# mlpc-ucsd/BDM

Hardware: AMD Instinct MI355X
Metric: sampled shapes/sec (4096 pts, 1000 DDPM steps) (higher is better)
Workload: dtype f32

## Files before the change

bdm_amd/csrc/dense_ops.hip:

```cpp
#include <stdlib.h>

#include "../../include/bdm_hip.h"
#include "common.h"
#include "se_fc.h"

using namespace bdm;
typedef __attribute__((ext_vector_type(16))) float f32x16;

#include "pointwise_common.h"

template <int MI, int NI, bool ATRANS = false, int BK = 16, bool FOLD = false>
__global__ __launch_bounds__(256) __attribute__((amdgpu_waves_per_eu(2))) void pw_gemm_kernel(int M, int K, int N, const float *__restrict__ W, int ldw,
                                                      long long bsw, const int *__restrict__ m_count,
                                                      const float *__restrict__ X, long long bsx, int ldx,
                                                      const float *__restrict__ bias,
                                                      const float *__restrict__ bbias, int ldbb,
                                                      const float *__restrict__ R, long long bsr, int ldr,
                                                      float *__restrict__ Y, long long bsy, int ldy, int act,
                                                      float slope, PwGn gn) {
  constexpr int BM = 32 * MI, BN = 128 * NI, LDA = BM + 4;
  __shared__ float As[BK * LDA];
  __shared__ __align__(16) float Bs[BK * BN];
  __shared__ float2 coef_s[FOLD ? 1024 : 1];
  const int tid = threadIdx.x, lane = tid & 63, wave = tid >> 6, li = lane & 31, lh = lane >> 5;
// ... 1042 lines not shown
  if (b == 0) return BDM_OK;
  if (workspace != nullptr) {
    const int p = sa_row_floats(c);
    BDM_REQUIRE((reinterpret_cast<size_t>(workspace) & 15) == 0, "sa_group: workspace must be 16-byte aligned");
    hipLaunchKernelGGL(sa_pack_points_kernel, dim3(cdiv(n, 256), cdiv(p / 4, 3), b), dim3(256), 0, (hipStream_t)stream, c, n, p,
                       coords, features, bs_f, ld_f, (float *)workspace);
    hipLaunchKernelGGL(sa_group_pm_kernel, dim3(cdiv(m * u, 256), cdiv(p / 4, SAQ), b), dim3(256), 0, (hipStream_t)stream, c,
                       n, m, u, p, (const float *)workspace, centers, indices, out);
    return launch_status("sa_group");
  }
  if (n >= 256 && n <= 8192 && (long long)m * u <= (1ll << 24)) {
    const int dma = (n % 256 == 0) && (ld_f % 4 == 0) && (bs_f % 4 == 0) && ((reinterpret_cast<size_t>(coords) & 15) == 0) &&
                    (c == 0 || (reinterpret_cast<size_t>(features) & 15) == 0);
    const size_t smem = sizeof(float) * SAG_R * (size_t)n + 1024;
    BDM_ALLOW_LDS(sa_group_lds_kernel, smem);
    hipLaunchKernelGGL(sa_group_lds_kernel, dim3(cdiv(c + 3, SAG_R), cdiv(m * u, SAG_EB), b), dim3(256), smem, (hipStream_t)stream, c, n, m, u,
                       dma, coords, centers, features, bs_f, ld_f, indices, out);
    return launch_status("sa_group");
  }
  int gy = c < 32 ? (c < 1 ? 1 : c) : 32;
  hipLaunchKernelGGL(sa_group_kernel, dim3(cdiv(m * u, 256), gy, b), dim3(256), 0, (hipStream_t)stream, c, n, m, u,
                     coords, centers, features, bs_f, ld_f, indices, out);
  return launch_status("sa_group");
}

__global__ void bcast_rows_kernel(int c, int l, const float *__restrict__ v, int ld_v, float *__restrict__ y,
                                  long long bs_y, int ld_y) {
  const int col = blockIdx.x * blockDim.x + threadIdx.x;
  const int bi = blockIdx.z;
  if (col >= l) return;
  for (int ci = blockIdx.y; ci < c; ci += gridDim.y)
    y[(size_t)bi * bs_y + (size_t)ci * ld_y + col] = v[(size_t)bi * ld_v + ci];
}
extern "C" int bdm_broadcast_rows(int b, int c, int l, const float *v, int ld_v, float *y, long long bs_y,
                                  int ld_y, void *stream) {
  BDM_REQUIRE(b >= 0 && c >= 1 && l >= 1, "broadcast_rows: bad sizes");
  if (b == 0) return BDM_OK;
  hipLaunchKernelGGL(bcast_rows_kernel, dim3(cdiv(l, 256), c < 64 ? c : 64, b), dim3(256), 0, (hipStream_t)stream, c,
                     l, v, ld_v, y, bs_y, ld_y);
  return launch_status("broadcast_rows");
}

__global__ void copy_rows_kernel(int c, int l, const float *__restrict__ x, long long bs_x, int ld_x,
                                 float *__restrict__ y, long long bs_y, int ld_y) {
  const int col = blockIdx.x * blockDim.x + threadIdx.x;
  const int bi = blockIdx.z;
// ... 682 lines not shown
```

bdm_amd/csrc/pvcnn_ops.hip:

```cpp
#include <stdarg.h>
#include <stdio.h>

#include <stdlib.h>

#include "../../include/bdm_hip.h"
#include "common.h"

#pragma clang fp contract(off)

namespace bdm {
static thread_local char g_err[512] = "";
void set_error(const char *fmt, ...) {
  va_list ap;
  va_start(ap, fmt);
  vsnprintf(g_err, sizeof(g_err), fmt, ap);
  va_end(ap);
}
}

extern "C" const char *bdm_last_error(void) { return bdm::g_err; }
extern "C" int bdm_abi_version(void) { return 4; }

using namespace bdm;

// ... 500 lines not shown
          __fadd_rn(__fadd_rn(__fmul_rn(fr[i0], w0), __fmul_rn(fr[i1], w1)), __fmul_rn(fr[i2], w2));
    } else if (ci < c_a + c_s) {
      out0[(size_t)bi * bs_0 + (size_t)ci * ld_0 + j] = fs[(size_t)bi * bs_s + (size_t)(ci - c_a) * ld_s + j];
    } else {
      const int ct = ci - c_a - c_s;
      const float *fr = ft + (size_t)bi * bs_t + (size_t)ct * ld_t;
      out1[(size_t)bi * bs_1 + (size_t)ct * ld_1 + j] =
          __fadd_rn(__fadd_rn(__fmul_rn(fr[i0], w0), __fmul_rn(fr[i1], w1)), __fmul_rn(fr[i2], w2));
    }
  }
}

extern "C" int bdm_fp_assemble(int b, int m, int n, const int *indices, const float *weights, int c_a, const float *fa,
                               long long bs_a, int ld_a, int c_s, const float *fs, long long bs_s, int ld_s, int c_t,
                               const float *ft, long long bs_t, int ld_t, float *out0, long long bs_0, int ld_0, float *out1,
                               long long bs_1, int ld_1, void *stream) {
  BDM_REQUIRE(b >= 0 && m >= 1 && n >= 0 && c_a >= 0 && c_s >= 0 && c_t >= 0, "fp_assemble: bad sizes");
  if (b == 0 || n == 0 || c_a + c_s + c_t == 0) return BDM_OK;
  const int c = c_a + c_s + c_t;
  dim3 grid(cdiv(n, 256), c < 64 ? c : 64, b);
  hipLaunchKernelGGL(fp_assemble_kernel, grid, dim3(256), 0, (hipStream_t)stream, n, c_a, fa, bs_a, ld_a, c_s, fs, bs_s, ld_s, c_t,
                     ft, bs_t, ld_t, indices, weights, out0, bs_0, ld_0, out1, bs_1, ld_1);
  return launch_status("fp_assemble");
}

extern "C" int bdm_three_nn_interpolate_forward(int b, int c, int m, int n, const float *points,
                                                const float *centers, const float *features, float *out,
                                                int *indices, float *weights, void *stream) {
  int rc = bdm_three_nn_search(b, m, n, points, centers, indices, weights, stream);
  if (rc) return rc;
  return bdm_three_nn_apply(b, c, m, n, features, (long long)c * m, m, indices, weights, out,
                            (long long)c * n, n, stream);
}

extern "C" size_t bdm_voxelize_workspace_bytes(int b, int n, int r) {
  return sizeof(int) * ((size_t)b * r * r * r + 2 * (size_t)b * n);
}

__global__ void vox_plan_kernel(int n, int r, const int *__restrict__ coords, int *__restrict__ ind,
                                int *__restrict__ cnt, int *__restrict__ start, int *__restrict__ tmp,
                                int *__restrict__ sorted, int n_max, int *__restrict__ occ_index,
                                int *__restrict__ occ_list, int *__restrict__ n_occ, unsigned char *__restrict__ rowocc) {
  extern __shared__ int lcnt[];
  __shared__ int wave_tot[16];
  const int r2 = r * r, r3 = r2 * r;
  const int bi = blockIdx.x, tid = threadIdx.x, T = blockDim.x, lane = tid & 63, wave = tid >> 6;
// ... 290 lines not shown
```

bdm_amd/modules.py:

```python
import os
from typing import NamedTuple

import torch
import torch.nn as nn

from . import functional as F
from . import ops
from . import tape

__all__ = ["Swish", "SharedMLP", "SE3d", "Voxelization", "Attention", "PVConv", "BallQuery",
           "PointNetSAModule", "PointNetFPModule"]


class Swish(nn.Module):

    def forward(self, x):
        raise RuntimeError("Swish is fused into bdm_group_norm on the HIP path")


class SharedMLP(nn.Module):

    def __init__(self, in_channels, out_channels, dim=1):
        super().__init__()
        if dim == 1:
            conv = nn.Conv1d
        elif dim == 2:
            conv = nn.Conv2d
        else:
            raise ValueError
        if not isinstance(out_channels, (list, tuple)):
            out_channels = [out_channels]
        layers = []
        for oc in out_channels:
            layers.extend([conv(in_channels, oc, 1), nn.GroupNorm(8, oc), Swish()])
            in_channels = oc
        self.layers = nn.Sequential(*layers)

    fold_gn = True

    def run(self, x, out_last=None, fold_last=False, x2=None, first_weight=None, first_add=None, first_bias=None):
        n = len(self.layers) // 3
        pending = None
        for i in range(n):
            conv, gn = self.layers[3 * i], self.layers[3 * i + 1]
            last = i == n - 1
            dst = out_last if last else None
            defer = (self.fold_gn and x.is_cuda and (not last or fold_last) and ops.gn_foldable(conv.out_channels, gn.num_groups))
            second = x2 if i == 0 else None
            weight = first_weight if (i == 0 and first_weight is not None) else conv.weight
            addend = first_add if i == 0 else None
            bb = first_bias if i == 0 else None
            if defer or pending is not None or second is not None or addend is not None or bb is not None:
                r = ops.pointwise_conv_gn(x, weight, conv.bias, out=dst, fold_in=pending,
                                          out_groups=gn.num_groups if defer else None, x2=second, add=addend, batch_bias=bb)
                if defer:
                    x, stats = r
                    pending = (stats, gn)
                else:
                    x, pending = r, None
                    ops.group_norm_(x, gn.weight, gn.bias, gn.num_groups, gn.eps, swish=True)
            else:
                x = ops.pointwise_conv(x, weight, conv.bias, out=dst)
                ops.group_norm_(x, gn.weight, gn.bias, gn.num_groups, gn.eps, swish=True)
        return (x, pending) if fold_last else x

    def forward(self, inputs):
        if isinstance(inputs, (list, tuple)):
            return (self.run(inputs[0]), *inputs[1:])
        return self.run(inputs)


def hoisted_first_weight(owner, conv, keep_cols):
    w = conv.weight
    hit = getattr(owner, "_hoist_w", None)
    if hit is None or hit[0] != (w._version, w.data_ptr(), keep_cols):
        w2 = w.detach().reshape(w.shape[0], -1)
        kept = w2[:, :keep_cols] if isinstance(keep_cols, int) else torch.cat([w2[:, lo:hi] for lo, hi in keep_cols], dim=1)
        hit = ((w._version, w.data_ptr(), keep_cols), kept.contiguous())
        owner._hoist_w = hit
    return hit[1]


class SE3d(nn.Module):

    def __init__(self, channel, reduction=8, use_relu=False):
        super().__init__()
        if not use_relu:
            raise NotImplementedError("the denoisers are built with with_se_relu=True (pvcnn_utils.py:93)")
        self.fc = nn.Sequential(nn.Linear(channel, channel // reduction, bias=False), nn.ReLU(True),
                                nn.Linear(channel // reduction, channel, bias=False), nn.Sigmoid())

    def gate(self, grid):
        return ops.se_gate(grid, self.fc[0].weight, self.fc[2].weight)


class Voxelization(nn.Module):

    def __init__(self, resolution, normalize=True, eps=0):
        super().__init__()
        self.r = int(resolution)
        self.normalize = normalize
        self.eps = eps
# ... 448 lines not shown
            radius = [radius]
        if not isinstance(num_neighbors, (list, tuple)):
            num_neighbors = [num_neighbors] * len(radius)
        assert len(radius) == len(num_neighbors)
        if not isinstance(out_channels, (list, tuple)):
            out_channels = [[out_channels]] * len(radius)
        elif not isinstance(out_channels[0], (list, tuple)):
            out_channels = [out_channels] * len(radius)
        assert len(radius) == len(out_channels)
        groupers, mlps = [], []
        total_out_channels = 0
        for _radius, _out_channels, _num_neighbors in zip(radius, out_channels, num_neighbors):
            groupers.append(BallQuery(radius=_radius, num_neighbors=_num_neighbors, include_coordinates=include_coordinates))
            mlps.append(SharedMLP(in_channels=in_channels + (3 if include_coordinates else 0),
                                  out_channels=_out_channels, dim=2))
            total_out_channels += _out_channels[-1]
        self.num_centers = num_centers
        self.out_channels = total_out_channels
        self.groupers = nn.ModuleList(groupers)
        self.mlps = nn.ModuleList(mlps)

    fuse_mlp = os.environ.get("BDM_SA_FUSED", "1") != "0"

    _temb_terms = None

    def temb_rows(self, c_t):
        w = self.mlps[0].layers[0].weight
        hit = getattr(self, "_temb_rows", None)
        if hit is None or hit[0] != (w._version, w.data_ptr(), c_t):
            w2 = w.detach().reshape(w.shape[0], -1)
            hit = ((w._version, w.data_ptr(), c_t), w2[:, w2.shape[1] - c_t:].contiguous())
            self._temb_rows = hit
        return hit[1]

    def can_split_temb(self, features, temb):
        conv0 = self.mlps[0].layers[0]
        return (PVConv.temb_split and features is not None and features.is_cuda and len(self.groupers) == 1
                and self.groupers[0].include_coordinates and ops.is_point_invariant(temb) and not ops.is_point_invariant(features)
                and 3 + features.shape[1] + temb.shape[1] == conv0.in_channels)

    def plan(self, coords):
        coords = coords.contiguous()
        centers_coords = self.sample(coords)
        return centers_coords, self.query(coords, centers_coords)

    def sample(self, coords):
# ... 6 lines not shown
    def forward(self, inputs):
        features, coords, temb = inputs
        coords = coords.contiguous()
        assert len(self.groupers) == 1, "multi-radius grouping is not used by the denoisers"
        planned = getattr(self, "_planned", None)
        self._planned = None
        if planned is not None and callable(planned[0]):
            planned = planned[0]() if planned[1] is coords else None
            self._planned = None
            if planned is None:
                self._more = None
        if planned is not None and planned[3] is coords:
            centers_coords, idx, event, _ = planned
            tape.wait_event(event)
            more, self._more = getattr(self, "_more", None), None
            if more is not None:
                more()
        else:
            centers_coords, idx = self.plan(coords)
        if (self.fuse_mlp and coords.is_cuda and features is not None and ops.is_point_invariant(temb) and idx.shape[1] <= 8192
                and ops.sa_mlp2_fusable(self.mlps[0], features.shape[1], idx.shape[2])):
            out = ops.sa_mlp2_fused(coords, centers_coords.contiguous(), features, idx, self.mlps[0])
            return out, centers_coords, temb[:, :, :1].expand(-1, -1, self.num_centers)
        grouped, g_t = self.groupers[0](coords, centers_coords, temb, features, neighbor_indices=idx)
        conv0 = self.mlps[0].layers[0]
        if grouped.shape[1] != conv0.in_channels:
            if not self.can_split_temb(features, temb):
                raise ValueError(f"PointNetSAModule's MLP expects {conv0.in_channels} grouped channels, got {grouped.shape[1]}")
            bb, self._temb_terms = self._temb_terms, None
            if bb is None or tuple(bb.shape) != (grouped.shape[0], conv0.out_channels):
                tvec = temb[:, :, 0].contiguous()
                bb = ops.pointwise_conv(tvec[:, :, None], self.temb_rows(temb.shape[1]))[:, :, 0]
            h, pending = self.mlps[0].run(grouped, fold_last=True, first_bias=bb,
                                          first_weight=hoisted_first_weight(self.mlps[0], conv0, grouped.shape[1]))
        else:
            h, pending = self.mlps[0].run(grouped, fold_last=True)
        out = ops.max_over_neighbors(h, fold=pending)
        if g_t.stride(2) == 0 and g_t.stride(3) == 0:
            temb_out = g_t[:, :, 0, 0][:, :, None].expand(-1, -1, self.num_centers)
        else:
            temb_out = ops.max_over_neighbors(g_t.contiguous())
        return out, centers_coords, temb_out


class PointNetFPModule(nn.Module):
    two_source = True
    _cond = None
    _temb_bias = None

    def temb_weight(self, c_feat, c_t):
        w = self.mlp.layers[0].weight
        hit = getattr(self, "_wt", None)
        if hit is None or hit[0] != (w._version, w.data_ptr(), c_feat, c_t):
            hit = ((w._version, w.data_ptr(), c_feat, c_t), w.detach().reshape(w.shape[0], -1)[:, c_feat:c_feat + c_t].contiguous())
            self._wt = hit
        return hit[1]

    def _need_skip(self, points_features):
        cond = self._cond
        if (cond is not None and not cond.features_ready and points_features is not None
                and points_features.data_ptr() == cond.x_cf[:, 3:].data_ptr()):
            cond.ensure_features()

    def can_split(self, centers_features, points_features, temb):
        conv0 = self.mlp.layers[0]
        c_skip = 0 if points_features is None else points_features.shape[1]
        return (centers_features.is_cuda and ops.is_point_invariant(temb) and not ops.is_point_invariant(centers_features)
                and centers_features.shape[1] + temb.shape[1] + c_skip == conv0.in_channels)

    def _forward_split(self, pc, cc, idx, w, features, points_features, temb, points_coords):
        from . import _lib as L
        B, _, n = pc.shape
        m, dev = cc.shape[2], pc.device
        conv0 = self.mlp.layers[0]
        c_feat, c_t = features.shape[1], temb.shape[1]
        c_skip = 0 if points_features is None else points_features.shape[1]
        bb, self._temb_bias = self._temb_bias, None
        if bb is None or tuple(bb.shape) != (B, conv0.out_channels):
            tvec = temb[:, :, 0].contiguous()
            bb = ops.pointwise_conv(tvec[:, :, None], self.temb_weight(c_feat, c_t))[:, :, 0]
        buf = torch.empty(B, c_feat, n, dtype=torch.float32, device=dev)
        fa, _, _, _, bs_a, ld_a = ops._bcl(features)
        _, _, _, _, bs_0, ld_0 = ops._bcl(buf)
        L.check(L.lib().bdm_fp_assemble(B, m, n, L.ptr(idx), L.ptr(w), c_feat, L.ptr(fa), L.c_ll(bs_a), ld_a, 0, None, L.c_ll(0), 0,
                                        0, None, L.c_ll(0), 0, L.ptr(buf), L.c_ll(bs_0), ld_0, None, L.c_ll(0), 0, L.stream()), "fp_assemble")
        temb = temb[:, :, :1].expand(-1, -1, n)
        if c_skip == 0:
            return self.mlp.run(buf, first_weight=hoisted_first_weight(self.mlp, conv0, c_feat), first_bias=bb), points_coords, temb
        cond = self._cond
        if cond is not None and points_features.shape[1] == cond.C and points_features.data_ptr() == cond.x_cf[:, 3:].data_ptr():
            fmap = cond.map("fp_skip", conv0.weight,
                            lambda conv=conv0, lo=c_feat + c_t, C=cond.C: conv.weight.detach().reshape(conv.out_channels, -1)[:, lo:lo + C])
            g = cond.gather(fmap)
            return (self.mlp.run(buf, first_weight=hoisted_first_weight(self.mlp, conv0, c_feat), first_add=g[:, 3:], first_bias=bb),
                    points_coords, temb)
        self._need_skip(points_features)
        keep = ((0, c_feat), (c_feat + c_t, c_feat + c_t + c_skip))
        return self.mlp.run(buf, x2=points_features, first_weight=hoisted_first_weight(self.mlp, conv0, keep), first_bias=bb), points_coords, temb

    def __init__(self, in_channels, out_channels):
        super().__init__()
        self.mlp = SharedMLP(in_channels=in_channels, out_channels=out_channels, dim=1)

# ... 3 lines not shown
            points_features = None
        else:
            points_coords, centers_coords, centers_features, points_features, temb = inputs
        from . import _lib as L
        pc, cc = points_coords.contiguous(), centers_coords.contiguous()
        B, _, n = pc.shape
        m = cc.shape[2]
        dev = pc.device
        from . import pvcnn
        planned = pvcnn.NN_PLANS.pop((pc.data_ptr(), cc.data_ptr()), None)
        if planned is not None and planned[0].shape == pc.shape and planned[1].shape == cc.shape:
            idx, w = planned[2], planned[3]
            tape.wait_event(planned[4])
        else:
            idx, w = ops.three_nn_search(pc, cc)

        c_t = temb.shape[1]
        if self.can_split(centers_features, points_features, temb):
            return self._forward_split(pc, cc, idx, w, centers_features, points_features, temb, points_coords)
        cf = ops.materialize(centers_features)
        c_int = cf.shape[1]
        c_skip = 0 if points_features is None else points_features.shape[1]
        two_source = self.two_source and c_skip > 0 and dev.type == "cuda"
        if two_source:
            skip_src, c_skip = points_features, 0
        buf = torch.empty(B, c_int + c_skip, n, dtype=torch.float32, device=dev)
        t_src = ops.materialize(temb)
        interpolated_temb = torch.empty(B, t_src.shape[1], n, dtype=torch.float32, device=dev)
        fa, _, _, _, bs_a, ld_a = ops._bcl(cf)
        ft, _, c_t, _, bs_t, ld_t = ops._bcl(t_src)
        if c_skip:
            self._need_skip(points_features)
            fs, _, _, _, bs_s, ld_s = ops._bcl(points_features)
        else:
            fs, bs_s, ld_s = None, 0, 0
        _, _, _, _, bs_0, ld_0 = ops._bcl(buf)
        _, _, _, _, bs_1, ld_1 = ops._bcl(interpolated_temb)
        L.check(L.lib().bdm_fp_assemble(B, m, n, L.ptr(idx), L.ptr(w), c_int, L.ptr(fa), L.c_ll(bs_a), ld_a, c_skip, L.ptr(fs),
                                        L.c_ll(bs_s), ld_s, c_t, L.ptr(ft), L.c_ll(bs_t), ld_t, L.ptr(buf), L.c_ll(bs_0), ld_0,
                                        L.ptr(interpolated_temb), L.c_ll(bs_1), ld_1, L.stream()), "fp_assemble")
        if two_source:
            cond = self._cond
            if (cond is not None and skip_src.shape[1] == cond.C and skip_src.data_ptr() == cond.x_cf[:, 3:].data_ptr()):
                conv = self.mlp.layers[0]
                fmap = cond.map("fp_skip", conv.weight,
                                lambda conv=conv, lo=c_int, C=cond.C: conv.weight.detach().reshape(conv.out_channels, -1)[:, lo:lo + C])
# ... 6 lines not shown
```

bdm_amd/ops.py:

```python
import ctypes
import os

import torch

from . import _lib as L
from . import tape


def _bcl(t):
    if t.dtype != torch.float32:
        raise L.BdmHipError(f"expected float32, got {t.dtype}")
    B, C = t.shape[0], t.shape[1]
    if B * C > 0 and t.is_contiguous():
        l = t.numel() // (B * C)
        return t, B, C, l, C * l, l
    l = 1
    for s in t.shape[2:]:
        l *= s
    dense, exp = True, 1
    for d in range(t.dim() - 1, 1, -1):
        if t.shape[d] != 1 and t.stride(d) != exp:
            dense = False
        exp *= t.shape[d]
    if dense and C > 1 and t.stride(1) < l:
# ... 171 lines not shown
        (p, slices, groups), gn = fold
        L.check(L.lib().bdm_max_over_neighbors_gn(B, C, M, U, L.ptr(x), L.ptr(p), slices, groups, L.ptr(gn.weight), L.ptr(gn.bias),
                                                  L.c_float(gn.eps), L.ptr(out), L.c_ll(bs_y), ld_y, L.stream()),
                "max_over_neighbors_gn")
        return out
    L.check(L.lib().bdm_max_over_neighbors(B, C, M, U, L.ptr(x), L.ptr(out), L.c_ll(bs_y), ld_y, L.stream()),
            "max_over_neighbors")
    return out


def sa_group(coords, centers, features, indices, point_major=None):
    B, _, n = coords.shape
    m, u = indices.shape[1], indices.shape[2]
    f, _, C, _, bs_f, ld_f = _bcl(features)
    out = torch.empty(B, 3 + C, m, u, dtype=torch.float32, device=coords.device)
    if point_major is None:
        point_major = B * m * u >= (1 << 18) and C <= 64
    ws = workspace(L.lib().bdm_sa_group_workspace_bytes(B, C, n), coords.device, "sa_group") if point_major else None
    L.check(L.lib().bdm_sa_group(B, C, n, m, u, L.ptr(coords), L.ptr(centers), L.ptr(f), L.c_ll(bs_f), ld_f,
                                 L.ptr(indices), L.ptr(out), L.ptr(ws), L.stream()), "sa_group")
    return out


def sa_mlp2_fusable(mlp, c_in, u):
    layers = mlp.layers
    if len(layers) != 6 or u != 32 or not 1 <= c_in <= 32:
        return False
    (c1, g1), (c2, g2) = (layers[0], layers[1]), (layers[3], layers[4])
    return (c1.out_channels == 32 and c2.out_channels == 64 and c1.in_channels == c_in + 3 and g1.num_groups == 8 and g2.num_groups == 8
            and c1.bias is not None and c2.bias is not None)


def sa_mlp2_fused(coords, centers, features, indices, mlp):
    B, _, n = coords.shape
    m, u = indices.shape[1], indices.shape[2]
    f, _, C, _, bs_f, ld_f = _bcl(features)
    dev = coords.device
    c1, g1, c2, g2 = mlp.layers[0], mlp.layers[1], mlp.layers[3], mlp.layers[4]
    rows = workspace(L.lib().bdm_sa_mlp2_fused_rows_bytes(B, C, n), dev, "sa_rows")
    S = L.lib().bdm_sa_mlp2_fused_slices(B, m)
    partial = torch.empty(2, B, 8, S, 2, dtype=torch.float64, device=dev)
    out = torch.empty(B, c2.out_channels, m, dtype=torch.float32, device=dev)
    _, _, _, _, bs_o, ld_o = _bcl(out)
    L.check(L.lib().bdm_sa_mlp2_fused(B, C, n, m, u, c1.out_channels, c2.out_channels, L.ptr(coords), L.ptr(f), L.c_ll(bs_f), ld_f,
                                      L.ptr(centers), L.ptr(indices), L.ptr(c1.weight), L.ptr(c1.bias), L.ptr(g1.weight), L.ptr(g1.bias),
                                      L.c_float(g1.eps), L.ptr(c2.weight), L.ptr(c2.bias), L.ptr(g2.weight), L.ptr(g2.bias),
# ... 1140 lines not shown
```

bdm_amd/profiling.py:

```python
import collections

import torch

from . import _lib as L

HBM_PEAK_GBS = 8000.0
MFMA16_PEAK_TFLOPS = 2500.0
MFMA32_PEAK_TFLOPS = 157.3
VALU_TESTS_PEAK = 1024 * 64 * 2.4e9 / 4 / 6.7 / 1e9
OCCUPANCY = {}
DILATED = {}


def _list_conv(a, which, products=3):
    b, cin, cout, r = a[0], a[1], a[2], a[3]
    dense = 2.0 * 27 * cin * cout * r ** 3 * b
    frac = DILATED.get(int(r), (1.0, 1.0))[which]
    return ("mfma_list", dense * frac, MFMA16_PEAK_TFLOPS / products, dense)


def _f(flops, products):
    return ("mfma", flops, MFMA16_PEAK_TFLOPS / products)


# ... 64 lines not shown
    "bdm_sparse_conv_rows_from_map": ("sparse first conv", lambda a: (a[0], a[1], a[2], a[4]), lambda a: ("hbm", 4.0 * a[0] * a[1] * a[4])),
    "bdm_sparse_voxel_features_s3": ("sparse first conv", lambda a: (a[0], a[1], a[2], a[3]), lambda a: ("hbm", 4.0 * a[0] * a[1] * a[2])),
    "bdm_sparse_voxel_features": ("sparse first conv", lambda a: (a[0], a[1], a[2], a[3]), lambda a: ("hbm", 4.0 * a[0] * a[1] * a[2])),
    "bdm_sparse_voxel_features_f32": ("sparse first conv", lambda a: (a[0], a[1], a[2], a[3]), lambda a: ("hbm", 4.0 * a[0] * a[1] * a[2])),
    "bdm_sparse_conv_fused": ("sparse first conv", lambda a: (a[0], a[1], a[2], a[3]), lambda a: ("hbm", 4.0 * a[0] * a[2] * a[3] ** 3)),
    "bdm_pointwise_conv": ("1x1 conv GEMM (fp32 MFMA)", lambda a: a[:4], _pw),
    "bdm_pointwise_conv_gn": ("1x1 conv GEMM (fp32 MFMA)", lambda a: a[:4], _pw),
    "bdm_pointwise_conv_gn_bb": ("1x1 conv GEMM (fp32 MFMA)", lambda a: a[:4], _pw),
    "bdm_pointwise_conv_gn_add": ("1x1 conv GEMM (fp32 MFMA)", lambda a: a[:4], _pw),
    "bdm_pointwise_conv_s3": ("1x1 conv GEMM (bf16x6)", lambda a: a[:4], _pw_s3),
    "bdm_pointwise_conv_gn_s3": ("1x1 conv GEMM (bf16x6)", lambda a: a[:4], _pw_s3),
    "bdm_group_norm": ("GroupNorm(+Swish)", lambda a: a[:4], lambda a: ("hbm", 8.0 * a[0] * a[1] * a[2])),
    "bdm_group_norm_to_h2": ("GroupNorm(+Swish)", lambda a: a[:4], lambda a: ("hbm", (4.0 + 4.0 + 4.0) * a[0] * a[1] * a[2])),
    "bdm_group_norm_to_h2_stats": ("GroupNorm(+Swish)", lambda a: a[:4], lambda a: ("hbm", (4.0 + 4.0) * a[0] * a[1] * a[2])),
    "bdm_group_norm_to_s3": ("GroupNorm(+Swish)", lambda a: a[:4], lambda a: ("hbm", (4.0 + 4.0 + 6.0) * a[0] * a[1] * a[2])),
    "bdm_attention_core": ("attention", lambda a: a[:3], _attn),
    "bdm_attention_core_h2": ("attention", lambda a: a[:3], lambda a: _f(4.0 * a[0] * a[1] * a[2] * a[2], 3)),
    "bdm_furthest_point_sampling": ("furthest point sampling", lambda a: a[:3], lambda a: ("hbm", 4.0 * a[0] * (3 * a[1] + 4 * a[2]))),
    "bdm_gather_features_forward": ("furthest point sampling", lambda a: a[:4], lambda a: ("hbm", 4.0 * a[0] * (2 * a[1] * a[3] + a[3]))),
    "bdm_ball_query": ("ball query (distance tests)", lambda a: (a[0], a[1], a[2], a[4]),
                       lambda a: ("valu", 1.0 * a[0] * a[1] * a[2], VALU_TESTS_PEAK, "G tests/s")),
    "bdm_sa_group": ("grouping gather + max over neighbours", lambda a: a[:5],
                     lambda a: ("hbm", 4.0 * a[0] * ((3 + a[1]) * a[2] + a[3] * a[4] + (a[1] + 3) * a[3] * a[4]))),
    "bdm_sa_mlp2_fused": ("1x1 conv GEMM (fp32 MFMA)", lambda a: a[:7],
                          lambda a: ("mfma", 2.0 * a[0] * a[3] * a[4] * ((3 + a[1]) * a[5] + a[5] * a[6]), MFMA32_PEAK_TFLOPS)),
    "bdm_grouping_forward": ("grouping gather + max over neighbours", lambda a: a[:5],
                             lambda a: ("hbm", 4.0 * a[0] * (a[1] * a[2] + a[3] * a[4] + a[1] * a[3] * a[4]))),
    "bdm_max_over_neighbors": ("grouping gather + max over neighbours", lambda a: a[:4], lambda a: ("hbm", 4.0 * a[0] * a[1] * a[2] * (a[3] + 1))),
    "bdm_max_over_neighbors_gn": ("grouping gather + max over neighbours", lambda a: a[:4], lambda a: ("hbm", 4.0 * a[0] * a[1] * a[2] * (a[3] + 1))),
    "bdm_three_nn_search": ("3-NN interpolation", lambda a: a[:3], lambda a: ("hbm", 4.0 * a[0] * (3 * a[2] + 3 * a[1] + 6 * a[2]))),
    "bdm_three_nn_apply": ("3-NN interpolation", lambda a: a[:4], lambda a: ("hbm", 4.0 * a[0] * (a[1] * a[2] + a[1] * a[3] + 6 * a[3]))),
    "bdm_fp_assemble": ("3-NN interpolation", lambda a: (a[0], a[1], a[2], a[5], a[9], a[13]),
                        lambda a: ("hbm", 4.0 * a[0] * ((a[5] + a[13]) * (a[1] + a[2]) + 2 * a[9] * a[2] + 6 * a[2]))),
    "bdm_voxelize_plan_full": ("voxelize / devoxelize", lambda a: a[:3], lambda a: ("hbm", 4.0 * a[0] * (4 * a[1] + 3 * a[2] ** 3))),
    "bdm_voxel_coords": ("voxelize / devoxelize", lambda a: a[:3], lambda a: ("hbm", 4.0 * a[0] * 9 * a[1])),
    "bdm_devoxelize_gate_add": ("voxelize / devoxelize", lambda a: a[:4], lambda a: ("hbm", 4.0 * a[0] * (3 * a[2] + 10 * a[1] * a[2]))),
    "bdm_se_gate_gn": ("SE gate", lambda a: (a[0], a[1], a[3]), lambda a: ("hbm", 4.0 * a[0] * a[1] * a[3])),
    "bdm_devoxelize_gn_gate_add": ("voxelize / devoxelize", lambda a: a[:4], lambda a: ("hbm", 4.0 * a[0] * (3 * a[2] + 10 * a[1] * a[2]))),
    "bdm_se_gate_gn_pf": ("SE gate", lambda a: (a[0], a[1], a[3]), lambda a: ("hbm", 4.0 * a[0] * a[1] * a[3])),
    "bdm_devoxelize_gn_gate_add_pf": ("voxelize / devoxelize", lambda a: a[:4], lambda a: ("hbm", 4.0 * a[0] * (3 * a[2] + 10 * a[1] * a[2]))),
    "bdm_devoxelize_gn_se_add": ("voxelize / devoxelize", lambda a: a[:4], lambda a: ("hbm", 4.0 * a[0] * (3 * a[2] + 10 * a[1] * a[2]))),
    "bdm_pvconv_tail_small": ("voxelize / devoxelize", lambda a: a[:4], lambda a: ("hbm", 4.0 * a[0] * (3 * a[2] + a[1] * a[3] ** 3 + 2 * a[1] * a[2]))),
    "bdm_sparse_conv_gather_h2_small": ("sparse first conv", lambda a: (a[0], a[1], a[2], a[3]), lambda a: ("hbm", 4.0 * a[0] * a[1] * a[2] ** 3)),
    "bdm_lincomb": ("scheduler step / blend", lambda a: a[:2], lambda a: ("hbm", 4.0 * a[0] * (a[1] + 1))),
    "bdm_se_gate": ("SE gate", lambda a: (a[0], a[1], a[3]), lambda a: ("hbm", 4.0 * a[0] * a[1] * a[3])),
    "bdm_copy_rows": ("concat / broadcast / transpose copies", lambda a: a[:3], lambda a: ("hbm", 8.0 * a[0] * a[1] * a[2])),
    "bdm_concat2_rows": ("concat / broadcast / transpose copies", lambda a: (a[0], a[1], a[2], a[6]), lambda a: ("hbm", 4.0 * a[0] * a[1] * (2 * a[2] + a[6]))),
    "bdm_broadcast_rows": ("concat / broadcast / transpose copies", lambda a: a[:3], lambda a: ("hbm", 4.0 * a[0] * a[1] * a[2])),
    "bdm_transpose": ("concat / broadcast / transpose copies", lambda a: a[:3], lambda a: ("hbm", 8.0 * a[0] * a[1] * a[2])),
    "bdm_rasterize_points": ("projection conditioning", lambda a: a[:4], lambda a: ("hbm", 4.0 * a[0] * 4 * a[1])),
    "bdm_condition_gather_cf": ("projection conditioning", lambda a: a[:4], lambda a: ("hbm", 4.0 * a[0] * a[1] * (2 * a[2] + 7))),
    "bdm_condition_xyz_cf": ("projection conditioning", lambda a: a[:3], lambda a: ("hbm", 4.0 * a[0] * a[1] * 6)),
    "bdm_condition_gather": ("projection conditioning", lambda a: a[:4], lambda a: ("hbm", 4.0 * a[0] * a[1] * (2 * a[2] + 7))),
    "bdm_ddpm_step": ("scheduler step / blend", lambda a: a[:1], lambda a: ("hbm", 16.0 * a[0])),
    "bdm_ddpm_step_philox": ("scheduler step / blend", lambda a: a[:2], lambda a: ("hbm", 12.0 * a[0] * a[1])),
    "bdm_pvd_step": ("scheduler step / blend", lambda a: a[:1], lambda a: ("hbm", 16.0 * a[0])),
# ... 170 lines not shown
```

include/bdm_hip.h:

```cpp
#ifndef BDM_HIP_H
#define BDM_HIP_H

#include <stddef.h>
#include <stdint.h>

#ifdef __cplusplus
extern "C" {
#endif

const char *bdm_last_error(void);
int bdm_abi_version(void);


int bdm_furthest_point_sampling(int b, int n, int m, const float *coords, int *indices,
                                float *centers_out, void *stream);

int bdm_gather_features_forward(int b, int c, int n, int m, const float *features,
                                const int *indices, float *out, void *stream);

int bdm_ball_query(int b, int n, int m, float radius, int u, const float *centers,
                   const float *points, int *neighbors, void *stream);

int bdm_grouping_forward(int b, int c, int n, int m, int u, const float *features,
                         const int *indices, float *out, void *stream);

int bdm_fp_assemble(int b, int m, int n, const int *indices, const float *weights, int c_a, const float *fa, long long bs_a,
                    int ld_a, int c_s, const float *fs, long long bs_s, int ld_s, int c_t, const float *ft, long long bs_t,
                    int ld_t, float *out0, long long bs_0, int ld_0, float *out1, long long bs_1, int ld_1, void *stream);
int bdm_three_nn_interpolate_forward(int b, int c, int m, int n, const float *points,
                                     const float *centers, const float *features, float *out,
                                     int *indices, float *weights, void *stream);
int bdm_three_nn_search(int b, int m, int n, const float *points, const float *centers,
                        int *indices, float *weights, void *stream);
int bdm_three_nn_apply(int b, int c, int m, int n, const float *features, long long bs_f, int ld_f,
                       const int *indices, const float *weights, float *out, long long bs_o, int ld_o,
                       void *stream);

size_t bdm_voxelize_workspace_bytes(int b, int n, int r);
int bdm_avg_voxelize_forward(int b, int c, int n, int r, const float *features, const int *coords,
                             float *out, int *ind, int *cnt, void *workspace, void *stream);

int bdm_trilinear_devoxelize_forward(int b, int c, int n, int r, const float *coords,
                                     const float *grid, float *out, void *stream);

int bdm_gather_features_backward(int b, int c, int n, int m, const float *grad_y, const int *indices,
                                 float *grad_x, void *stream);
int bdm_grouping_backward(int b, int c, int n, int m, int u, const float *grad_y, const int *indices,
                          float *grad_x, void *stream);
int bdm_three_nn_interpolate_backward(int b, int c, int n, int m, const float *grad_y, const int *indices,
                                      const float *weights, float *grad_x, void *stream);
int bdm_trilinear_devoxelize_backward(int b, int c, int n, int r, const int *inds, const float *wgts,
// ... 35 lines not shown

#ifdef BDM_EXPERIMENTAL
size_t bdm_pointwise_s3_weight_elems(int m, int k);
int bdm_pointwise_s3_pack_weights(int m, int k, const float *w, int ldw, void *packed, void *stream);
int bdm_pointwise_conv_s3(int b, int m, int k, int n, const void *packed_w, const float *x, long long bs_x, int ld_x,
                          const float *bias, const float *batch_bias, int ld_bb, const float *residual, long long bs_r,
                          int ld_r, float *y, long long bs_y, int ld_y, int act, float slope, void *stream);
int bdm_pointwise_conv_gn_s3(int b, int m, int k, int n, const void *packed_w, const float *x, long long bs_x, int ld_x,
                             const float *x2, long long bs_x2, int ld_x2, int k1, const float *bias, float *y, long long bs_y,
                             int ld_y, const void *in_partial, int in_slices, int in_groups, const float *in_gamma,
                             const float *in_beta, float in_eps, int out_groups, void *out_partial, float *amax,
                             int amax_rows, void *stream);
#endif
int bdm_max_over_neighbors_gn(int b, int c, int m, int u, const float *x, const void *in_partial, int in_slices, int groups,
                              const float *gamma, const float *beta, float eps, float *y, long long bs_y, int ld_y,
                              void *stream);
int bdm_max_over_neighbors(int b, int c, int m, int u, const float *x, float *y, long long bs_y,
                           int ld_y, void *stream);

size_t bdm_sa_group_workspace_bytes(int b, int c, int n);
int bdm_sa_group(int b, int c, int n, int m, int u, const float *coords, const float *centers,
                 const float *features, long long bs_f, int ld_f, const int *indices, float *out,
                 void *workspace, void *stream);

size_t bdm_sa_mlp2_fused_rows_bytes(int b, int c, int n);
int bdm_sa_mlp2_fused_slices(int b, int m);
int bdm_sa_mlp2_fused(int b, int c, int n, int m, int u, int m1, int m2, const float *coords, const float *features,
                      long long bs_f, int ld_f, const float *centers, const int *indices, const float *w1, const float *b1,
                      const float *g1w, const float *g1b, float eps1, const float *w2, const float *b2, const float *g2w,
                      const float *g2b, float eps2, int groups, void *rows, void *partial1, void *partial2, float *out,
                      long long bs_o, int ld_o, void *stream);

int bdm_broadcast_rows(int b, int c, int l, const float *v, int ld_v, float *y, long long bs_y,
                       int ld_y, void *stream);
int bdm_concat2_rows(int b, int l, int c0, const float *x0, long long bs_0, int ld_0, int c1, const float *x1, long long bs_1,
                     int ld_1, float *y, long long bs_y, int ld_y, void *stream);
int bdm_copy_rows(int b, int c, int l, const float *x, long long bs_x, int ld_x, float *y,
                  long long bs_y, int ld_y, void *stream);
int bdm_transpose(int b, int rows, int cols, const float *x, float *y, void *stream);

int bdm_time_embedding(int b, int dim, const float *t, const float *w0, const float *b0,
                       const float *w2, const float *b2, float *out, void *stream);
int bdm_time_embedding_i64(int b, int dim, const long long *t, const float *w0, const float *b0,
                           const float *w2, const float *b2, float *out, void *stream);

int bdm_voxel_coords(int b, int n, int r, float eps, const float *coords, float *norm_coords,
// ... 284 lines not shown
```

Baseline: 3.042.

## Commute first 1x1 conv before gather/interpolation in SA and FP modules

Adds kernels that apply the first pointwise conv to the source points before grouping (SA) or 3-NN interpolation (FP), then gather and combine the pre-activations with the coordinate term, bias and GroupNorm partial statistics. Because the gather and the interpolation are linear, the GEMM can run on the smaller source set instead of the expanded neighbour or upsampled set. FP commuting is on by default; SA commuting is opt-in through an environment variable. The cost is extra kernels and a change in floating-point summation order.

```diff
diff --git a/bdm_amd/csrc/dense_ops.hip b/bdm_amd/csrc/dense_ops.hip
--- a/bdm_amd/csrc/dense_ops.hip
+++ b/bdm_amd/csrc/dense_ops.hip
@@ -1088,6 +1088,119 @@
   hipLaunchKernelGGL(sa_group_kernel, dim3(cdiv(m * u, 256), gy, b), dim3(256), 0, (hipStream_t)stream, c, n, m, u,
                      coords, centers, features, bs_f, ld_f, indices, out);
   return launch_status("sa_group");
+}
+
+constexpr int SGP_EB = 4096;
+static inline int sgp_rows(int cg) { return (cg % 8 == 0) ? 8 : 4; }
+template <int R, bool STAGED>
+__global__ __launch_bounds__(256) void sa_group_preact_kernel(int c_out, int n, int m, int u, const float *__restrict__ coords,
+                                                              const float *__restrict__ centers, const float *__restrict__ P, long long bs_p,
+                                                              int ld_p, const float *__restrict__ wxyz, int ldw, const float *__restrict__ bias,
+                                                              const float *__restrict__ bbias, int ld_bb, const int *__restrict__ idx,
+                                                              float *__restrict__ y, double *__restrict__ partial, int cg, int S) {
+  extern __shared__ __align__(16) float sgp_tile[];
+  __shared__ double sgp_red[4][2];
+  const int bi = blockIdx.z, ch0 = blockIdx.x * R;
+  const int lane = threadIdx.x & 63, wave = threadIdx.x >> 6;
+  const size_t mu = (size_t)m * u;
+  const float *pc = coords + (size_t)bi * 3 * n;
+  const float *pb = P + (size_t)bi * bs_p + (size_t)ch0 * ld_p;
+  if constexpr (STAGED) {
+    const int ppr = n >> 8;
+    for (int q = wave; q < (3 + R) * ppr; q += 4) {
+      const int r = q / ppr, p = q - r * ppr;
+      const float *g = (r < 3 ? pc + (size_t)r * n : pb + (size_t)(r - 3) * ld_p) + p * 256 + lane * 4;
+      __builtin_amdgcn_global_load_lds((const __attribute__((address_space(1))) void *)g,
+                                       (__attribute__((address_space(3))) void *)(sgp_tile + (size_t)r * n + p * 256), 16, 0, 0);
+    }
+  }
+  float wx[R], wy[R], wz[R], cst[R];
+#pragma unroll
+  for (int r = 0; r < R; ++r) {
+    const float *wr = wxyz + (size_t)(ch0 + r) * ldw;
+    wx[r] = wr[0]; wy[r] = wr[1]; wz[r] = wr[2];
+    cst[r] = (bias ? bias[ch0 + r] : 0.f) + (bbias ? bbias[(size_t)bi * ld_bb + ch0 + r] : 0.f);
+  }
+  const int e0 = blockIdx.y * SGP_EB, e1 = (int)min((size_t)e0 + SGP_EB, mu);
+  const int *ib = idx + (size_t)bi * mu;
+  int src[SGP_EB / 256];
+#pragma unroll
+  for (int k = 0; k < SGP_EB / 256; ++k) {
+    const int e = e0 + threadIdx.x + k * 256;
+    src[k] = e < e1 ? min(max(ib[e], 0), n - 1) : 0;
+  }
+  if constexpr (STAGED) __syncthreads();
+  float *ob = y + ((size_t)bi * c_out + ch0) * mu;
+  const float *cc = centers + (size_t)bi * 3 * m;
+  double s = 0.0, q = 0.0;
+#pragma unroll 4
+  for (int k = 0; k < SGP_EB / 256; ++k) {
+    const int e = e0 + threadIdx.x + k * 256;
+    if (e < e1) {
+      const int j = src[k], i = e / u;
+      float px, py, pz, v[R];
+      if constexpr (STAGED) {
+        px = sgp_tile[j]; py = sgp_tile[(size_t)n + j]; pz = sgp_tile[2 * (size_t)n + j];
+#pragma unroll
+        for (int r = 0; r < R; ++r) v[r] = sgp_tile[(size_t)(3 + r) * n + j];
+      } else {
+        px = pc[j]; py = pc[(size_t)n + j]; pz = pc[2 * (size_t)n + j];
+#pragma unroll
+        for (int r = 0; r < R; ++r) v[r] = pb[(size_t)r * ld_p + j];
+      }
+      const float dx = px - cc[i], dy = py - cc[(size_t)m + i], dz = pz - cc[2 * (size_t)m + i];
+#pragma unroll
+      for (int r = 0; r < R; ++r) {
+        const float o = (v[r] + (wx[r] * dx + wy[r] * dy + wz[r] * dz)) + cst[r];
+        ob[(size_t)r * mu + e] = o;
+        s += (double)o;
+        q += (double)o * (double)o;
+      }
+    }
+  }
+  if (partial != nullptr) {
+    s = wave_sum(s); q = wave_sum(q);
+    if (lane == 0) { sgp_red[wave][0] = s; sgp_red[wave][1] = q; }
+    __syncthreads();
+    if (threadIdx.x < 2) {
+      const int t = threadIdx.x, G = c_out / cg, g = ch0 / cg, sl = ((ch0 % cg) / R) * gridDim.y + blockIdx.y;
+      partial[(((size_t)bi * G + g) * S + sl) * 2 + t] = ((sgp_red[0][t] + sgp_red[1][t]) + sgp_red[2][t]) + sgp_red[3][t];
+    }
+  }
+}
+
+extern "C" int bdm_sa_group_preact_slices(int c_out, int m, int u, int groups) {
+  if (groups < 1 || c_out % groups || (c_out / groups) % 4) return 0;
+  const int cg = c_out / groups;
+  return (cg / sgp_rows(cg)) * (int)cdivll((long long)m * u, SGP_EB);
+}
+
+extern "C" int bdm_sa_group_preact(int b, int c_out, int n, int m, int u, const float *coords, const float *centers, const float *p,
+                                   long long bs_p, int ld_p, const float *w_xyz, int ldw, const float *bias, const float *batch_bias,
+                                   int ld_bb, const int *indices, float *y, int groups, void *out_partial, void *stream) {
+  BDM_REQUIRE(b >= 0 && c_out >= 4 && n >= 1 && m >= 1 && u >= 1 && ldw >= 3, "sa_group_preact: bad sizes");
+  BDM_REQUIRE((long long)m * u <= (1ll << 24) && (long long)c_out * ld_p + n < (1ll << 31), "sa_group_preact: shape too large");
+  BDM_REQUIRE(coords && centers && p && w_xyz && indices && y, "sa_group_preact: null argument");
+  const int G = groups >= 1 ? groups : 1;
+  BDM_REQUIRE(c_out % G == 0 && (c_out / G) % 4 == 0, "sa_group_preact: channels per group must be a multiple of 4 (c_out=%d groups=%d)",
+              c_out, groups);
+  BDM_REQUIRE(out_partial == nullptr || groups >= 1, "sa_group_preact: statistics need groups >= 1");
+  if (b == 0) return BDM_OK;
+  const int cg = c_out / G, R = sgp_rows(cg), S = (cg / R) * cdiv(m * u, SGP_EB);
+  const bool staged = n >= 256 && n <= 2048 && (n % 256 == 0) && (ld_p % 4 == 0) && (bs_p % 4 == 0) &&
+                      ((reinterpret_cast<size_t>(coords) & 15) == 0) && ((reinterpret_cast<size_t>(p) & 15) == 0);
+  const dim3 grid(c_out / R, cdiv(m * u, SGP_EB), b);
+#define SGP_LAUNCH(RR, ST)                                                                                                         \
+  do {                                                                                                                             \
+    const size_t smem = ST ? sizeof(float) * (3 + RR) * (size_t)n + 1024 : 0;                                                      \
+    BDM_ALLOW_LDS((sa_group_preact_kernel<RR, ST>), smem);                                                                         \
+    hipLaunchKernelGGL((sa_group_preact_kernel<RR, ST>), grid, dim3(256), smem, (hipStream_t)stream, c_out, n, m, u, coords,       \
+                       centers, p, bs_p, ld_p, w_xyz, ldw, bias, batch_bias, ld_bb, indices, y, (double *)out_partial, cg, S);     \
+  } while (0)
+  if (R == 8) { if (staged) SGP_LAUNCH(8, true); else SGP_LAUNCH(8, false); }
+  else        { if (staged) SGP_LAUNCH(4, true); else SGP_LAUNCH(4, false); }
+#undef SGP_LAUNCH
+  return launch_status("sa_group_preact");
 }
 
 __global__ void bcast_rows_kernel(int c, int l, const float *__restrict__ v, int ld_v, float *__restrict__ y,
diff --git a/bdm_amd/csrc/pvcnn_ops.hip b/bdm_amd/csrc/pvcnn_ops.hip
--- a/bdm_amd/csrc/pvcnn_ops.hip
+++ b/bdm_amd/csrc/pvcnn_ops.hip
@@ -546,6 +546,79 @@
   hipLaunchKernelGGL(fp_assemble_kernel, grid, dim3(256), 0, (hipStream_t)stream, n, c_a, fa, bs_a, ld_a, c_s, fs, bs_s, ld_s, c_t,
                      ft, bs_t, ld_t, indices, weights, out0, bs_0, ld_0, out1, bs_1, ld_1);
   return launch_status("fp_assemble");
+}
+
+constexpr int FPP_R = 4;
+constexpr int FPP_EB = 1024;
+__global__ __launch_bounds__(256) void fp_interp_preact_kernel(int c_out, int m, int n, const int *__restrict__ indices,
+                                                               const float *__restrict__ weights, const float *__restrict__ P, long long bs_p,
+                                                               int ld_p, const float *__restrict__ add, long long bs_a, int ld_a,
+                                                               const float *__restrict__ bias, const float *__restrict__ bbias, int ld_bb,
+                                                               float *__restrict__ y, long long bs_y, int ld_y, double *__restrict__ partial,
+                                                               int cg, int S) {
+  __shared__ double red[4][2];
+  const int bi = blockIdx.z, ch0 = blockIdx.x * FPP_R;
+  const int lane = threadIdx.x & 63, wave = threadIdx.x >> 6;
+  const int *id = indices + (size_t)bi * 3 * n;
+  const float *w = weights + (size_t)bi * 3 * n;
+  const float *pb = P + (size_t)bi * bs_p + (size_t)ch0 * ld_p;
+  const float *ab = add ? add + (size_t)bi * bs_a + (size_t)ch0 * ld_a : nullptr;
+  float *ob = y + (size_t)bi * bs_y + (size_t)ch0 * ld_y;
+  float cst[FPP_R];
+#pragma unroll
+  for (int r = 0; r < FPP_R; ++r) cst[r] = __fadd_rn(bias ? bias[ch0 + r] : 0.f, bbias ? bbias[(size_t)bi * ld_bb + ch0 + r] : 0.f);
+  double s = 0.0, q = 0.0;
+  const int e1 = min((int)(blockIdx.y + 1) * FPP_EB, n);
+#pragma unroll
+  for (int k = 0; k < FPP_EB / 256; ++k) {
+    const int j = blockIdx.y * FPP_EB + threadIdx.x + k * 256;
+    if (j < e1) {
+      const int i0 = min(max(id[j], 0), m - 1), i1 = min(max(id[n + j], 0), m - 1), i2 = min(max(id[2 * n + j], 0), m - 1);
+      const float w0 = w[j], w1 = w[n + j], w2 = w[2 * n + j];
+#pragma unroll
+      for (int r = 0; r < FPP_R; ++r) {
+        const float *fr = pb + (size_t)r * ld_p;
+        float o = __fadd_rn(__fadd_rn(__fmul_rn(fr[i0], w0), __fmul_rn(fr[i1], w1)), __fmul_rn(fr[i2], w2));
+        if (ab) o = __fadd_rn(o, ab[(size_t)r * ld_a + j]);
+        o = __fadd_rn(o, cst[r]);
+        ob[(size_t)r * ld_y + j] = o;
+        s += (double)o;
+        q += (double)o * (double)o;
+      }
+    }
+  }
+  if (partial != nullptr) {
+    s = wave_sum(s); q = wave_sum(q);
+    if (lane == 0) { red[wave][0] = s; red[wave][1] = q; }
+    __syncthreads();
+    if (threadIdx.x < 2) {
+      const int t = threadIdx.x, G = c_out / cg, g = ch0 / cg, sl = ((ch0 % cg) / FPP_R) * gridDim.y + blockIdx.y;
+      partial[(((size_t)bi * G + g) * S + sl) * 2 + t] = ((red[0][t] + red[1][t]) + red[2][t]) + red[3][t];
+    }
+  }
+}
+
+extern "C" int bdm_fp_interp_preact_slices(int c_out, int n, int groups) {
+  if (groups < 1 || c_out % groups || (c_out / groups) % FPP_R) return 0;
+  return (c_out / groups / FPP_R) * cdiv(n, FPP_EB);
+}
+
+extern "C" int bdm_fp_interp_preact(int b, int c_out, int m, int n, const int *indices, const float *weights, const float *p,
+                                    long long bs_p, int ld_p, const float *add, long long bs_add, int ld_add, const float *bias,
+                                    const float *batch_bias, int ld_bb, float *y, long long bs_y, int ld_y, int groups,
+                                    void *out_partial, void *stream) {
+  BDM_REQUIRE(b >= 0 && c_out >= FPP_R && m >= 1 && n >= 0, "fp_interp_preact: bad sizes");
+  BDM_REQUIRE(indices && weights && p && y, "fp_interp_preact: null argument");
+  const int G = groups >= 1 ? groups : 1;
+  BDM_REQUIRE(c_out % G == 0 && (c_out / G) % FPP_R == 0, "fp_interp_preact: channels per group must be a multiple of 4 (c_out=%d groups=%d)",
+              c_out, groups);
+  BDM_REQUIRE(out_partial == nullptr || groups >= 1, "fp_interp_preact: statistics need groups >= 1");
+  if (b == 0 || n == 0) return BDM_OK;
+  const int cg = c_out / G, S = (cg / FPP_R) * cdiv(n, FPP_EB);
+  hipLaunchKernelGGL(fp_interp_preact_kernel, dim3(c_out / FPP_R, cdiv(n, FPP_EB), b), dim3(256), 0, (hipStream_t)stream, c_out, m, n,
+                     indices, weights, p, bs_p, ld_p, add, bs_add, ld_add, bias, batch_bias, ld_bb, y, bs_y, ld_y,
+                     (double *)out_partial, cg, S);
+  return launch_status("fp_interp_preact");
 }
 
 extern "C" int bdm_three_nn_interpolate_forward(int b, int c, int m, int n, const float *points,
diff --git a/bdm_amd/modules.py b/bdm_amd/modules.py
--- a/bdm_amd/modules.py
+++ b/bdm_amd/modules.py
@@ -38,10 +38,19 @@
 
     fold_gn = True
 
-    def run(self, x, out_last=None, fold_last=False, x2=None, first_weight=None, first_add=None, first_bias=None):
+    def run(self, x, out_last=None, fold_last=False, x2=None, first_weight=None, first_add=None, first_bias=None, first_done=None):
         n = len(self.layers) // 3
         pending = None
-        for i in range(n):
+        start = 0
+        if first_done is not None:
+            x, stats = first_done
+            gn = self.layers[1]
+            if stats is not None and (n > 1 or fold_last):
+                pending = (stats, gn)
+            else:
+                ops.group_norm_(x, gn.weight, gn.bias, gn.num_groups, gn.eps, swish=True)
+            start = 1
+        for i in range(start, n):
             conv, gn = self.layers[3 * i], self.layers[3 * i + 1]
             last = i == n - 1
             dst = out_last if last else None
@@ -78,6 +87,16 @@
         kept = w2[:, :keep_cols] if isinstance(keep_cols, int) else torch.cat([w2[:, lo:hi] for lo, hi in keep_cols], dim=1)
         hit = ((w._version, w.data_ptr(), keep_cols), kept.contiguous())
         owner._hoist_w = hit
+    return hit[1]
+
+
+def weight_columns(owner, conv, lo, hi):
+    w = conv.weight
+    cache = owner.__dict__.setdefault("_wcols", {})
+    hit = cache.get((lo, hi))
+    if hit is None or hit[0] != (w._version, w.data_ptr()):
+        hit = ((w._version, w.data_ptr()), w.detach().reshape(w.shape[0], -1)[:, lo:hi].contiguous())
+        cache[(lo, hi)] = hit
     return hit[1]
 
 
@@ -572,6 +591,29 @@
 
     fuse_mlp = os.environ.get("BDM_SA_FUSED", "1") != "0"
 
+    commute_first = os.environ.get("BDM_COMMUTE_FIRST_SA", "0") == "1"
+
+    def commutes_first(self, features, temb, m, u):
+        if not (self.commute_first and features is not None and features.is_cuda and features.shape[1] >= 1 and len(self.groupers) == 1
+                and self.groupers[0].include_coordinates and m * u > features.shape[2]):
+            return False
+        conv0, gn0 = self.mlps[0].layers[0], self.mlps[0].layers[1]
+        if not (SharedMLP.fold_gn and ops.gn_foldable(conv0.out_channels, gn0.num_groups)):
+            return False
+        return 3 + features.shape[1] == conv0.in_channels or self.can_split_temb(features, temb)
+
+    def _first_layer_commuted(self, coords, centers_coords, features, temb, idx):
+        conv0, gn0 = self.mlps[0].layers[0], self.mlps[0].layers[1]
+        C, bb = features.shape[1], None
+        if 3 + C != conv0.in_channels:
+            bb, self._temb_terms = self._temb_terms, None
+            if bb is None or tuple(bb.shape) != (features.shape[0], conv0.out_channels):
+                tvec = temb[:, :, 0].contiguous()
+                bb = ops.pointwise_conv(tvec[:, :, None], self.temb_rows(temb.shape[1]))[:, :, 0]
+        p = ops.pointwise_conv(features, weight_columns(self.mlps[0], conv0, 3, 3 + C))
+        return ops.sa_group_preact(coords, centers_coords.contiguous(), p, weight_columns(self.mlps[0], conv0, 0, 3), conv0.bias, bb,
+                                   idx, groups=gn0.num_groups)
+
     _temb_terms = None
 
     def temb_rows(self, c_t):
@@ -624,6 +666,12 @@
                 and ops.sa_mlp2_fusable(self.mlps[0], features.shape[1], idx.shape[2])):
             out = ops.sa_mlp2_fused(coords, centers_coords.contiguous(), features, idx, self.mlps[0])
             return out, centers_coords, temb[:, :, :1].expand(-1, -1, self.num_centers)
+        if self.commutes_first(features, temb, idx.shape[1], idx.shape[2]):
+            h, pending = self.mlps[0].run(None, fold_last=True, first_done=self._first_layer_commuted(coords, centers_coords, features, temb, idx))
+            out = ops.max_over_neighbors(h, fold=pending)
+            if ops.is_point_invariant(temb):
+                return out, centers_coords, temb[:, :, :1].expand(-1, -1, self.num_centers)
+            return out, centers_coords, ops.max_over_neighbors(F.grouping(temb, idx).contiguous())
         grouped, g_t = self.groupers[0](coords, centers_coords, temb, features, neighbor_indices=idx)
         conv0 = self.mlps[0].layers[0]
         if grouped.shape[1] != conv0.in_channels:
@@ -670,6 +718,28 @@
         return (centers_features.is_cuda and ops.is_point_invariant(temb) and not ops.is_point_invariant(centers_features)
                 and centers_features.shape[1] + temb.shape[1] + c_skip == conv0.in_channels)
 
+    commute_first = os.environ.get("BDM_COMMUTE_FIRST_FP", "1") != "0"
+
+    def commutes_first(self, centers_features, n):
+        conv0, gn0 = self.mlp.layers[0], self.mlp.layers[1]
+        return bool(self.commute_first and centers_features.is_cuda and SharedMLP.fold_gn and n > centers_features.shape[2]
+                    and ops.gn_foldable(conv0.out_channels, gn0.num_groups))
+
+    def _first_layer_commuted(self, idx, w, features, n, points_features, skip_lo, bb):
+        conv0, gn0 = self.mlp.layers[0], self.mlp.layers[1]
+        p = ops.pointwise_conv(features, weight_columns(self.mlp, conv0, 0, features.shape[1]))
+        add = None
+        if points_features is not None and points_features.shape[1] > 0:
+            cond, c_skip = self._cond, points_features.shape[1]
+            if cond is not None and c_skip == cond.C and points_features.data_ptr() == cond.x_cf[:, 3:].data_ptr():
+                fmap = cond.map("fp_skip", conv0.weight,
+                                lambda conv=conv0, lo=skip_lo, C=cond.C: conv.weight.detach().reshape(conv.out_channels, -1)[:, lo:lo + C])
+                add = cond.gather(fmap)[:, 3:]
+            else:
+                self._need_skip(points_features)
+                add = ops.pointwise_conv(points_features, weight_columns(self.mlp, conv0, skip_lo, skip_lo + c_skip))
+        return ops.fp_interp_preact(idx, w, p, n, add=add, bias=conv0.bias, batch_bias=bb, groups=gn0.num_groups)
+
     def _forward_split(self, pc, cc, idx, w, features, points_features, temb, points_coords):
         from . import _lib as L
         B, _, n = pc.shape
@@ -681,6 +751,9 @@
         if bb is None or tuple(bb.shape) != (B, conv0.out_channels):
             tvec = temb[:, :, 0].contiguous()
             bb = ops.pointwise_conv(tvec[:, :, None], self.temb_weight(c_feat, c_t))[:, :, 0]
+        if self.commutes_first(features, n):
+            done = self._first_layer_commuted(idx, w, features, n, points_features, c_feat + c_t, bb)
+            return self.mlp.run(None, first_done=done), points_coords, temb[:, :, :1].expand(-1, -1, n)
         buf = torch.empty(B, c_feat, n, dtype=torch.float32, device=dev)
         fa, _, _, _, bs_a, ld_a = ops._bcl(features)
         _, _, _, _, bs_0, ld_0 = ops._bcl(buf)
@@ -730,6 +803,16 @@
         c_int = cf.shape[1]
         c_skip = 0 if points_features is None else points_features.shape[1]
         two_source = self.two_source and c_skip > 0 and dev.type == "cuda"
+        if (two_source or c_skip == 0) and self.commutes_first(cf, n):
+            t_src = ops.materialize(temb)
+            interpolated_temb = torch.empty(B, t_src.shape[1], n, dtype=torch.float32, device=dev)
+            ft, _, c_t, _, bs_t, ld_t = ops._bcl(t_src)
+            _, _, _, _, bs_1, ld_1 = ops._bcl(interpolated_temb)
+            L.check(L.lib().bdm_fp_assemble(B, m, n, L.ptr(idx), L.ptr(w), 0, None, L.c_ll(0), 0, 0, None, L.c_ll(0), 0, c_t, L.ptr(ft),
+                                            L.c_ll(bs_t), ld_t, None, L.c_ll(0), 0, L.ptr(interpolated_temb), L.c_ll(bs_1), ld_1,
+                                            L.stream()), "fp_assemble")
+            done = self._first_layer_commuted(idx, w, cf, n, points_features, c_int, None)
+            return self.mlp.run(None, first_done=done), points_coords, interpolated_temb
         if two_source:
             skip_src, c_skip = points_features, 0
         buf = torch.empty(B, c_int + c_skip, n, dtype=torch.float32, device=dev)
diff --git a/bdm_amd/ops.py b/bdm_amd/ops.py
--- a/bdm_amd/ops.py
+++ b/bdm_amd/ops.py
@@ -217,6 +217,55 @@
     return out
 
 
+def _preact_stats(slices, B, groups, device, what):
+    if slices <= 0:
+        raise L.BdmHipError(f"{what}: GroupNorm({groups}) statistics are not available for this width")
+    return torch.empty(B * groups * slices * 2, dtype=torch.float64, device=device), slices, groups
+
+
+def sa_group_preact(coords, centers, p, w_xyz, bias, batch_bias, indices, groups=None):
+    B, _, n = coords.shape
+    m, u = indices.shape[1], indices.shape[2]
+    pp, Bp, M, n_p, bs_p, ld_p = _bcl(p)
+    assert pp.data_ptr() == p.data_ptr() and (Bp, n_p) == (B, n) and tuple(w_xyz.shape) == (M, 3) and w_xyz.stride(1) == 1
+    y = torch.empty(B, M, m, u, dtype=torch.float32, device=coords.device)
+    lib = L.lib()
+    stats = _preact_stats(lib.bdm_sa_group_preact_slices(M, m, u, int(groups)), B, int(groups), coords.device, "sa_group_preact") if groups else None
+    bb, ld_bb = None, 0
+    if batch_bias is not None:
+        bb = batch_bias.reshape(B, -1)
+        assert bb.shape[1] == M and bb.stride(1) == 1, "batch_bias must be (B, M) with unit channel stride"
+        ld_bb = bb.stride(0)
+    L.check(lib.bdm_sa_group_preact(B, M, n, m, u, L.ptr(coords), L.ptr(centers), L.ptr(p), L.c_ll(bs_p), ld_p, L.ptr(w_xyz), w_xyz.stride(0),
+                                    L.ptr(bias), L.ptr(bb), ld_bb, L.ptr(indices), L.ptr(y), int(groups or 0),
+                                    L.ptr(stats[0]) if stats else None, L.stream()), "sa_group_preact")
+    return (y, stats) if groups else y
+
+
+def fp_interp_preact(indices, weights, p, n, add=None, bias=None, batch_bias=None, groups=None):
+    pp, B, M, m, bs_p, ld_p = _bcl(p)
+    assert pp.data_ptr() == p.data_ptr() and tuple(indices.shape) == (B, 3, n) and tuple(weights.shape) == (B, 3, n)
+    assert indices.is_contiguous() and weights.is_contiguous()
+    y = torch.empty(B, M, n, dtype=torch.float32, device=p.device)
+    _, _, _, _, bs_y, ld_y = _bcl(y)
+    lib = L.lib()
+    stats = _preact_stats(lib.bdm_fp_interp_preact_slices(M, n, int(groups)), B, int(groups), p.device, "fp_interp_preact") if groups else None
+    ap, bs_a, ld_a = None, 0, 0
+    if add is not None:
+        aa, Ba, Ma, na, bs_a, ld_a = _bcl(add)
+        assert aa.data_ptr() == add.data_ptr() and (Ba, Ma, na) == (B, M, n), "add must be a dense-row (B, M, n) view"
+        ap = add
+    bb, ld_bb = None, 0
+    if batch_bias is not None:
+        bb = batch_bias.reshape(B, -1)
+        assert bb.shape[1] == M and bb.stride(1) == 1, "batch_bias must be (B, M) with unit channel stride"
+        ld_bb = bb.stride(0)
+    L.check(lib.bdm_fp_interp_preact(B, M, m, n, L.ptr(indices), L.ptr(weights), L.ptr(p), L.c_ll(bs_p), ld_p, L.ptr(ap), L.c_ll(bs_a), ld_a,
+                                     L.ptr(bias), L.ptr(bb), ld_bb, L.ptr(y), L.c_ll(bs_y), ld_y, int(groups or 0),
+                                     L.ptr(stats[0]) if stats else None, L.stream()), "fp_interp_preact")
+    return (y, stats) if groups else y
+
+
 def sa_mlp2_fusable(mlp, c_in, u):
     layers = mlp.layers
     if len(layers) != 6 or u != 32 or not 1 <= c_in <= 32:
diff --git a/bdm_amd/profiling.py b/bdm_amd/profiling.py
--- a/bdm_amd/profiling.py
+++ b/bdm_amd/profiling.py
@@ -110,6 +110,8 @@
                        lambda a: ("valu", 1.0 * a[0] * a[1] * a[2], VALU_TESTS_PEAK, "G tests/s")),
     "bdm_sa_group": ("grouping gather + max over neighbours", lambda a: a[:5],
                      lambda a: ("hbm", 4.0 * a[0] * ((3 + a[1]) * a[2] + a[3] * a[4] + (a[1] + 3) * a[3] * a[4]))),
+    "bdm_sa_group_preact": ("grouping gather + max over neighbours", lambda a: a[:5],
+                            lambda a: ("hbm", 4.0 * a[0] * ((3 + a[1]) * a[2] + a[3] * a[4] + a[1] * a[3] * a[4]))),
     "bdm_sa_mlp2_fused": ("1x1 conv GEMM (fp32 MFMA)", lambda a: a[:7],
                           lambda a: ("mfma", 2.0 * a[0] * a[3] * a[4] * ((3 + a[1]) * a[5] + a[5] * a[6]), MFMA32_PEAK_TFLOPS)),
     "bdm_grouping_forward": ("grouping gather + max over neighbours", lambda a: a[:5],
@@ -120,6 +122,8 @@
     "bdm_three_nn_apply": ("3-NN interpolation", lambda a: a[:4], lambda a: ("hbm", 4.0 * a[0] * (a[1] * a[2] + a[1] * a[3] + 6 * a[3]))),
     "bdm_fp_assemble": ("3-NN interpolation", lambda a: (a[0], a[1], a[2], a[5], a[9], a[13]),
                         lambda a: ("hbm", 4.0 * a[0] * ((a[5] + a[13]) * (a[1] + a[2]) + 2 * a[9] * a[2] + 6 * a[2]))),
+    "bdm_fp_interp_preact": ("3-NN interpolation", lambda a: a[:4],
+                             lambda a: ("hbm", 4.0 * a[0] * (a[1] * (a[2] + a[3] * (2 if a[9] else 1)) + 6 * a[3]))),
     "bdm_voxelize_plan_full": ("voxelize / devoxelize", lambda a: a[:3], lambda a: ("hbm", 4.0 * a[0] * (4 * a[1] + 3 * a[2] ** 3))),
     "bdm_voxel_coords": ("voxelize / devoxelize", lambda a: a[:3], lambda a: ("hbm", 4.0 * a[0] * 9 * a[1])),
     "bdm_devoxelize_gate_add": ("voxelize / devoxelize", lambda a: a[:4], lambda a: ("hbm", 4.0 * a[0] * (3 * a[2] + 10 * a[1] * a[2]))),
diff --git a/include/bdm_hip.h b/include/bdm_hip.h
--- a/include/bdm_hip.h
+++ b/include/bdm_hip.h
@@ -27,6 +27,10 @@
 int bdm_fp_assemble(int b, int m, int n, const int *indices, const float *weights, int c_a, const float *fa, long long bs_a,
                     int ld_a, int c_s, const float *fs, long long bs_s, int ld_s, int c_t, const float *ft, long long bs_t,
                     int ld_t, float *out0, long long bs_0, int ld_0, float *out1, long long bs_1, int ld_1, void *stream);
+int bdm_fp_interp_preact_slices(int c_out, int n, int groups);
+int bdm_fp_interp_preact(int b, int c_out, int m, int n, const int *indices, const float *weights, const float *p, long long bs_p,
+                         int ld_p, const float *add, long long bs_add, int ld_add, const float *bias, const float *batch_bias,
+                         int ld_bb, float *y, long long bs_y, int ld_y, int groups, void *out_partial, void *stream);
 int bdm_three_nn_interpolate_forward(int b, int c, int m, int n, const float *points,
                                      const float *centers, const float *features, float *out,
                                      int *indices, float *weights, void *stream);
@@ -108,6 +112,11 @@
 int bdm_sa_group(int b, int c, int n, int m, int u, const float *coords, const float *centers,
                  const float *features, long long bs_f, int ld_f, const int *indices, float *out,
                  void *workspace, void *stream);
+
+int bdm_sa_group_preact_slices(int c_out, int m, int u, int groups);
+int bdm_sa_group_preact(int b, int c_out, int n, int m, int u, const float *coords, const float *centers, const float *p,
+                        long long bs_p, int ld_p, const float *w_xyz, int ldw, const float *bias, const float *batch_bias, int ld_bb,
+                        const int *indices, float *y, int groups, void *out_partial, void *stream);
 
 size_t bdm_sa_mlp2_fused_rows_bytes(int b, int c, int n);
 int bdm_sa_mlp2_fused_slices(int b, int m);
```

Result: no change. 3.059, median of 6 (+0.5%).
